# amorim-cleison/sign-language-nlp

Measured on AMD Instinct MI355X. Metric: train seq/s (batch=50,len=48), higher is better.
Workload: dtype bf16x3; 1 GPU; cfg2: Transformer train step E512 H8 N6 F512 batch 50 len 48 |src| 3000 |tgt| 202 dropout 0.1, fwd+CE+bwd+clip(0.5)+SGD(m=.9); launch=eager stream launches (auto: timed both in 9 untimed pre-warmup steps + warmup), per_gpu=independent fit (grid shard)

## Files before the change

sign-language-nlp_amd/csrc/elementwise.hip:

```cpp
#include "common.hpp"
#include "launch.hpp"
#include "layernorm_row.hpp"

namespace slnlp {

__device__ __forceinline__ void embed_fwd_body(const long* __restrict__ ids, long ld_ids, int B, int S,
                                                        int E, int V, const float* __restrict__ table,
                                                        const float* __restrict__ pe, float* __restrict__ out,
                                                        float scale, float drop_p, unsigned drop_thr, int drop_site,
                                                        const unsigned long long* __restrict__ rng, long nan_idx,
                                                        PlaneOut po, unsigned char* __restrict__ keep_mask) {
    const int e4 = E >> 2;
    const long total = (long)B * S * e4;
    const float ik = 1.f / (1.f - drop_p);
    for (long idx = blockIdx.x * 256L + threadIdx.x; idx < total; idx += (long)gridDim.x * 256) {
        const int m = (int)(idx / e4), c = (int)(idx % e4) * 4;
        const int s = m / B, b = m % B;
        const long id = ids[(long)b * ld_ids + s];
        float4 v = make_float4(0.f, 0.f, 0.f, 0.f);
        if (id >= 0 && id < V) v = *reinterpret_cast<const float4*>(table + id * E + c);
        const float4 p = pe ? *reinterpret_cast<const float4*>(pe + (long)s * E + c) : make_float4(0.f, 0.f, 0.f, 0.f);
        v.x = v.x * scale + p.x; v.y = v.y * scale + p.y; v.z = v.z * scale + p.z; v.w = v.w * scale + p.w;
        if (drop_p > 0.f) {
            const bool k0 = dropout_keep(rng, drop_site, m, c + 0, drop_thr), k1 = dropout_keep(rng, drop_site, m, c + 1, drop_thr);
            const bool k2 = dropout_keep(rng, drop_site, m, c + 2, drop_thr), k3 = dropout_keep(rng, drop_site, m, c + 3, drop_thr);
            v.x = k0 ? v.x * ik : 0.f; v.y = k1 ? v.y * ik : 0.f; v.z = k2 ? v.z * ik : 0.f; v.w = k3 ? v.w * ik : 0.f;
            if (keep_mask) keep_mask[idx] = (unsigned char)((k0 ? 1 : 0) | (k1 ? 2 : 0) | (k2 ? 4 : 0) | (k3 ? 8 : 0));
        }
        if (id == nan_idx) v = make_float4(NAN, NAN, NAN, NAN);
        *reinterpret_cast<float4*>(out + (long)m * E + c) = v;
        store_planes4(po, (long)m * E + c, v);
    }
}
SLNLP_ZKERNEL(embed_fwd_kernel, 256, embed_fwd_body)

__device__ __forceinline__ float4 load_dx_row(const float* __restrict__ dx, int t, int E, int c, float drop_p,
                                              float ik, unsigned thr, int site,
                                              const unsigned long long* __restrict__ rng,
                                              const unsigned char* __restrict__ keep_mask) {
    float4 g = *reinterpret_cast<const float4*>(dx + (long)t * E + c);
    if (drop_p > 0.f && keep_mask) {
        const unsigned k = keep_mask[((long)t * E + c) >> 2];
        g.x = (k & 1u) ? g.x * ik : 0.f; g.y = (k & 2u) ? g.y * ik : 0.f;
        g.z = (k & 4u) ? g.z * ik : 0.f; g.w = (k & 8u) ? g.w * ik : 0.f;
    } else if (drop_p > 0.f) {
        g.x = dropout_keep(rng, site, t, c + 0, thr) ? g.x * ik : 0.f;
        g.y = dropout_keep(rng, site, t, c + 1, thr) ? g.y * ik : 0.f;
        g.z = dropout_keep(rng, site, t, c + 2, thr) ? g.z * ik : 0.f;
        g.w = dropout_keep(rng, site, t, c + 3, thr) ? g.w * ik : 0.f;
    }
    return g;
}

constexpr int EMB_CHUNK = 64;

__device__ __forceinline__ void embed_bwd_chunk_body(const long* __restrict__ ids, long ld_ids, int B, int S,
                                                              int E, int V, const float* __restrict__ dx,
                                                              float* __restrict__ partial, int* __restrict__ pid,
                                                              float drop_p, unsigned drop_thr, int drop_site,
                                                              const unsigned long long* __restrict__ rng,
                                                              const unsigned char* __restrict__ keep_mask) {
    const int M = B * S, lane = threadIdx.x & 63;
    const int m = blockIdx.x, m0 = (m / EMB_CHUNK) * EMB_CHUNK, t = m - m0, mine = m0 + lane;
    int my_id = -1;
    if (mine < M) {
        const long v = ids[(long)(mine % B) * ld_ids + (mine / B)];
        my_id = (v < 0 || v >= V) ? -1 : (int)v;
    }
    const float ik = 1.f / (1.f - drop_p);
    const int id = __builtin_amdgcn_readlane(my_id, __builtin_amdgcn_readfirstlane(t));
    const unsigned long long mask = __ballot(my_id == id && id >= 0);
    const bool first = id >= 0 && (mask & ((1ull << t) - 1ull)) == 0ull;
    if (threadIdx.x == 0) pid[m] = first ? id : -1;
    if (!first) return;
    __shared__ __attribute__((aligned(16))) float red[4][256];
    const int wave = threadIdx.x >> 6;
    const unsigned long long wmask = mask & (0xFFFFull << (16 * wave));
    for (int c0 = 0; c0 < E; c0 += 256) {
        const int c = c0 + lane * 4;
        float4 acc = make_float4(0.f, 0.f, 0.f, 0.f);
        if (c < E) {
            unsigned long long bits = wmask;
            while (bits) {
                int k[4];
#pragma unroll
                for (int u = 0; u < 4; ++u) {
                    k[u] = bits ? __ffsll((long long)bits) - 1 : -1;
                    bits &= bits - 1;
                }
                float4 g[4];
#pragma unroll
                for (int u = 0; u < 4; ++u)
                    g[u] = k[u] >= 0 ? load_dx_row(dx, m0 + k[u], E, c, drop_p, ik, drop_thr, drop_site, rng, keep_mask)
                                     : make_float4(0.f, 0.f, 0.f, 0.f);
#pragma unroll
                for (int u = 0; u < 4; ++u) { acc.x += g[u].x; acc.y += g[u].y; acc.z += g[u].z; acc.w += g[u].w; }
            }
        }
        if (c0 > 0) __syncthreads();
        *reinterpret_cast<float4*>(&red[wave][lane * 4]) = acc;
        __syncthreads();
        if (wave == 0 && c < E) {
            float4 r = *reinterpret_cast<const float4*>(&red[0][lane * 4]);
#pragma unroll
            for (int w = 1; w < 4; ++w) {
                const float4 q = *reinterpret_cast<const float4*>(&red[w][lane * 4]);
                r.x += q.x; r.y += q.y; r.z += q.z; r.w += q.w;
            }
            *reinterpret_cast<float4*>(partial + (long)m * E + c) = r;
        }
    }
}
SLNLP_ZKERNEL(embed_bwd_chunk_kernel, 256, embed_bwd_chunk_body)

__device__ __forceinline__ void embed_bwd_combine_body(const int* __restrict__ pid, int M, int E,
                                                                const float* __restrict__ partial,
                                                                float* __restrict__ dtable, float scale) {
    __shared__ int list[1024];
    __shared__ int nlist;
    const int m = blockIdx.x, tid = threadIdx.x;
    const int id = pid[m];
    if (id < 0) return;
    int dup = 0;
    for (int mm = tid; mm < m; mm += 256) dup |= (pid[mm] == id);
    if (__syncthreads_or(dup)) return;
    if (tid == 0) nlist = 0;
    __syncthreads();
    for (int base = m; base < M; base += 256) {
        const int mm = base + tid;
        const bool hit = mm < M && pid[mm] == id;
        const unsigned long long bal = __ballot(hit);
        __shared__ unsigned long long match[4];
        __syncthreads();
        if ((tid & 63) == 0) match[tid >> 6] = bal;
        __syncthreads();
        if (tid == 0) {
            int n = nlist;
            for (int w = 0; w < 4; ++w) {
                unsigned long long bits = match[w];
                while (bits && n < 1024) {
                    list[n++] = base + w * 64 + __ffsll((long long)bits) - 1;
                    bits &= bits - 1;
                }
            }
            nlist = n;
        }
        __syncthreads();
    }
    const int n = nlist;
    __shared__ __attribute__((aligned(16))) float red[4][256];
    const int wave = tid >> 6, lane = tid & 63, per = (n + 3) / 4;
    const int i0 = wave * per, i1 = (i0 + per < n) ? i0 + per : n;
    for (int c0 = 0; c0 < E; c0 += 256) {
        const int c = c0 + lane * 4;
        float4 acc = make_float4(0.f, 0.f, 0.f, 0.f);
        if (c < E) {
            for (int i = i0; i < i1; i += 4) {
                float4 g[4];
#pragma unroll
                for (int u = 0; u < 4; ++u)
                    g[u] = (i + u < i1) ? *reinterpret_cast<const float4*>(partial + (long)list[i + u] * E + c)
                                        : make_float4(0.f, 0.f, 0.f, 0.f);
#pragma unroll
                for (int u = 0; u < 4; ++u) { acc.x += g[u].x; acc.y += g[u].y; acc.z += g[u].z; acc.w += g[u].w; }
            }
        }
        if (c0 > 0) __syncthreads();
        *reinterpret_cast<float4*>(&red[wave][lane * 4]) = acc;
        __syncthreads();
        if (wave == 0 && c < E) {
            float4 r = *reinterpret_cast<const float4*>(&red[0][lane * 4]);
#pragma unroll
            for (int w = 1; w < 4; ++w) {
                const float4 q = *reinterpret_cast<const float4*>(&red[w][lane * 4]);
                r.x += q.x; r.y += q.y; r.z += q.z; r.w += q.w;
            }
            r.x *= scale; r.y *= scale; r.z *= scale; r.w *= scale;
            *reinterpret_cast<float4*>(dtable + (long)id * E + c) = r;
        }
    }
}
SLNLP_ZKERNEL(embed_bwd_combine_kernel, 256, embed_bwd_combine_body)

__device__ __forceinline__ void embed_bwd_small_body(const long* __restrict__ ids, long ld_ids, int B, int S, int E, int V,
                                                     const float* __restrict__ dx, float* __restrict__ dtable, float scale,
                                                     float drop_p, unsigned drop_thr, int drop_site,
                                                     const unsigned long long* __restrict__ rng) {
    const int M = B * S, lane = threadIdx.x & 63, m = blockIdx.x;
    int my_id = -1;
    if (lane < M) {
        const long v = ids[(long)(lane % B) * ld_ids + (lane / B)];
        my_id = (v < 0 || v >= V) ? -1 : (int)v;
    }
    if (m < V && __ballot(my_id == m) == 0ull) {
        for (int c = threadIdx.x * 4; c < E; c += 1024) *reinterpret_cast<float4*>(dtable + (long)m * E + c) = make_float4(0.f, 0.f, 0.f, 0.f);
    }
    if (m >= M) return;
    const float ik = 1.f / (1.f - drop_p);
    const int id = __builtin_amdgcn_readlane(my_id, __builtin_amdgcn_readfirstlane(m));
    const unsigned long long mask = __ballot(my_id == id && id >= 0);
    const bool first = id >= 0 && (mask & ((1ull << m) - 1ull)) == 0ull;
    if (!first) return;
    __shared__ __attribute__((aligned(16))) float red[4][256];
    const int wave = threadIdx.x >> 6;
    const unsigned long long wmask = mask & (0xFFFFull << (16 * wave));
    for (int c0 = 0; c0 < E; c0 += 256) {
        const int c = c0 + lane * 4;
        float4 acc = make_float4(0.f, 0.f, 0.f, 0.f);
        if (c < E) {
            unsigned long long bits = wmask;
            while (bits) {
                int k[4];
#pragma unroll
                for (int u = 0; u < 4; ++u) {
                    k[u] = bits ? __ffsll((long long)bits) - 1 : -1;
                    bits &= bits - 1;
                }
                float4 g[4];
#pragma unroll
                for (int u = 0; u < 4; ++u)
                    g[u] = k[u] >= 0 ? load_dx_row(dx, k[u], E, c, drop_p, ik, drop_thr, drop_site, rng, nullptr)
                                     : make_float4(0.f, 0.f, 0.f, 0.f);
#pragma unroll
                for (int u = 0; u < 4; ++u) { acc.x += g[u].x; acc.y += g[u].y; acc.z += g[u].z; acc.w += g[u].w; }
            }
        }
        if (c0 > 0) __syncthreads();
        *reinterpret_cast<float4*>(&red[wave][lane * 4]) = acc;
        __syncthreads();
        if (wave == 0 && c < E) {
            float4 r = *reinterpret_cast<const float4*>(&red[0][lane * 4]);
#pragma unroll
            for (int w = 1; w < 4; ++w) {
                const float4 q = *reinterpret_cast<const float4*>(&red[w][lane * 4]);
                r.x += q.x; r.y += q.y; r.z += q.z; r.w += q.w;
            }
            r.x *= scale; r.y *= scale; r.z *= scale; r.w *= scale;
            *reinterpret_cast<float4*>(dtable + (long)id * E + c) = r;
        }
    }
}
SLNLP_ZKERNEL(embed_bwd_small_kernel, 256, embed_bwd_small_body)

int embed_fwd(const int64_t* ids, int64_t ld_ids, int B, int S, int E, int V, const float* table, const float* pe,
              float* out, float scale, float drop_p, int drop_site, const unsigned long long* rng, int64_t nan_idx,
              hipStream_t st, PlaneOut po, unsigned char* keep_mask) {
    SLNLP_CHECK_ARG(ids && table && out, "embed_fwd: null pointer");
    SLNLP_CHECK_ARG(B > 0 && S > 0 && V > 0 && E > 0 && E % 4 == 0, "embed_fwd: bad shape B=%d S=%d E=%d V=%d", B, S, E, V);
    SLNLP_CHECK_ARG(drop_p >= 0.f && drop_p < 1.f && (drop_p == 0.f || rng), "embed_fwd: bad dropout args");
    const long total = (long)B * S * (E / 4);
    int grid = ceil_div(total, 256);
    if (grid > 2048) grid = 2048;
    SLNLP_TRY(zlaunch(embed_fwd_kernel, dim3(grid), 256, 0, st, "embed_fwd",
                      (const long*)ids, (long)ld_ids, B, S, E, V, table, pe, out, scale, drop_p, dropout_threshold(drop_p), drop_site, rng, (long)nan_idx, po, keep_mask));
    return 0;
}

size_t embed_bwd_scratch_bytes(int B, int S, int E) {
    return ((size_t)B * S * E * sizeof(float) + (size_t)B * S * sizeof(int) + 255) & ~(size_t)255;
}

int embed_bwd(const int64_t* ids, int64_t ld_ids, int B, int S, int E, int V, const float* dx, float* dtable,
              float scale, int64_t zero_row, float drop_p, int drop_site, const unsigned long long* rng, void* scratch,
              hipStream_t st, const unsigned char* keep_mask) {
    SLNLP_CHECK_ARG(ids && dx && dtable && scratch, "embed_bwd: null pointer");
    SLNLP_CHECK_ARG(B > 0 && S > 0 && V > 0 && E > 0 && E % 4 == 0, "embed_bwd: bad shape");
    SLNLP_CHECK_ARG((long)B * S <= 65536, "embed_bwd: more than 65536 tokens per batch");
    SLNLP_CHECK_ARG(drop_p >= 0.f && drop_p < 1.f && (drop_p == 0.f || rng), "embed_bwd: bad dropout args");
    const int M = B * S;
    if (M <= EMB_CHUNK && !keep_mask) {
        SLNLP_TRY(zlaunch(embed_bwd_small_kernel, dim3(M > V ? M : V), 256, 0, st, "embed_bwd_small",
                          (const long*)ids, (long)ld_ids, B, S, E, V, dx, dtable, scale, drop_p, dropout_threshold(drop_p), drop_site, rng));
        if (zero_row >= 0 && zero_row < V) SLNLP_TRY(fill_zero(dtable + zero_row * E, (size_t)E * sizeof(float), st));
        return 0;
    }
    SLNLP_TRY(fill_zero(dtable, (size_t)V * E * sizeof(float), st));
    float* partial = (float*)scratch;
    int* pid = (int*)(partial + (size_t)M * E);
    SLNLP_TRY(zlaunch(embed_bwd_chunk_kernel, dim3(M), 256, 0, st, "embed_bwd_chunk",
                      (const long*)ids, (long)ld_ids, B, S, E, V, dx, partial, pid, drop_p, dropout_threshold(drop_p), drop_site, rng, keep_mask));
    SLNLP_TRY(zlaunch(embed_bwd_combine_kernel, dim3(M), 256, 0, st, "embed_bwd_combine",
                      pid, M, E, partial, dtable, scale));
    if (zero_row >= 0 && zero_row < V) SLNLP_TRY(fill_zero(dtable + zero_row * E, (size_t)E * sizeof(float), st));
    return 0;
}


__device__ __forceinline__ void layernorm_fwd_body(const float* __restrict__ x,
                                                            const float* __restrict__ gamma,
                                                            const float* __restrict__ beta, int rows, int E,
                                                            float eps, float* __restrict__ y,
                                                            float* __restrict__ stats, PlaneOut po) {
    const int lane = threadIdx.x & 63, wave = threadIdx.x >> 6;
    const int row = blockIdx.x * 4 + wave;
    if (row >= rows) return;
    const float* xr = x + (long)row * E;
    float4 v[LN_MAXU], g[LN_MAXU], bt[LN_MAXU];
#pragma unroll
    for (int u = 0; u < LN_MAXU; ++u) {
        const int c = lane * 4 + u * 256;
        const bool in = c < E;
        v[u] = in ? *reinterpret_cast<const float4*>(xr + c) : make_float4(0.f, 0.f, 0.f, 0.f);
        g[u] = in ? *reinterpret_cast<const float4*>(gamma + c) : make_float4(0.f, 0.f, 0.f, 0.f);
        bt[u] = in ? *reinterpret_cast<const float4*>(beta + c) : make_float4(0.f, 0.f, 0.f, 0.f);
    }
    float mean, rstd;
    layernorm_row(v, g, bt, E, eps, lane, mean, rstd, [&](int, int c, const float4& o) {
        *reinterpret_cast<float4*>(y + (long)row * E + c) = o;
        store_planes4(po, (long)row * E + c, o);
    });
    if (lane == 0 && stats) {
        stats[2 * row] = mean;
        stats[2 * row + 1] = rstd;
    }
}
SLNLP_ZKERNEL(layernorm_fwd_kernel, 256, layernorm_fwd_body)

template <int U, int GS, int RB, bool FUSE>
__device__ __forceinline__ void layernorm_bwd_rows(
    const float* __restrict__ dy, const float* __restrict__ x, const float* __restrict__ gamma,
    const float* __restrict__ stats, int rows, int E, const float* __restrict__ add_to_dx, float* __restrict__ dx,
    float* __restrict__ dx_drop, float drop_p, unsigned drop_thr, int drop_site,
    const unsigned long long* __restrict__ rng, PlaneOut po_dx, PlaneOut po_drop, float* __restrict__ partial, int chunk_rows, int nchunks) {
    const int lane = threadIdx.x & 63, wave = threadIdx.x >> 6;
    const float invE = 1.f / (float)E, ik = 1.f / (1.f - drop_p);
    const bool want_drop = dx_drop != nullptr || po_drop.hi != nullptr;
    const bool drop = want_drop && drop_p > 0.f;
    const int unit = FUSE ? (int)blockIdx.x : blockIdx.x * (int)(blockDim.x >> 6) + wave;
    float4 ag[U], ab[U];
#pragma unroll
    for (int u = 0; u < U; ++u) ag[u] = ab[u] = make_float4(0.f, 0.f, 0.f, 0.f);
    const int row_begin = FUSE ? unit * chunk_rows + wave * GS : unit * GS;
    const int row_end = FUSE ? ((unit + 1) * chunk_rows < rows ? (unit + 1) * chunk_rows : rows) : row_begin + GS;
    const int row_step = FUSE ? 4 * GS : GS;
    if (!FUSE && row_begin >= rows) return;
    DropKey dkey = {};
    if (drop) dkey = dropout_key(rng, drop_site);
    float4 g[U];
#pragma unroll
    for (int u = 0; u < U; ++u)
        if (lane * 4 + u * 256 < E) g[u] = *reinterpret_cast<const float4*>(gamma + lane * 4 + u * 256);
#pragma unroll 1
    for (int row0 = row_begin; row0 < row_end; row0 += row_step)
#pragma unroll
    for (int i0 = 0; i0 < GS; i0 += RB) {
        float4 d[RB][U], v[RB][U];
        float mean[RB], rstd[RB], s1[RB], s2[RB];
#pragma unroll
        for (int i = 0; i < RB; ++i) {
            const int row = row0 + i0 + i < rows ? row0 + i0 + i : rows - 1;
            mean[i] = stats[2 * row];
            rstd[i] = stats[2 * row + 1];
#pragma unroll
            for (int u = 0; u < U; ++u) {
                const int c = lane * 4 + u * 256;
                if (c < E) {
                    d[i][u] = *reinterpret_cast<const float4*>(dy + (long)row * E + c);
                    v[i][u] = *reinterpret_cast<const float4*>(x + (long)row * E + c);
                }
            }
        }
#pragma unroll
        for (int i = 0; i < RB; ++i) {
            float a1 = 0.f, a2 = 0.f;
#pragma unroll
            for (int u = 0; u < U; ++u) {
                if (lane * 4 + u * 256 < E) {
                    const float4 dd = d[i][u], vv = v[i][u];
                    const float4 xh = make_float4((vv.x - mean[i]) * rstd[i], (vv.y - mean[i]) * rstd[i], (vv.z - mean[i]) * rstd[i], (vv.w - mean[i]) * rstd[i]);
                    const float4 gv = make_float4(dd.x * g[u].x, dd.y * g[u].y, dd.z * g[u].z, dd.w * g[u].w);
                    a1 += gv.x + gv.y + gv.z + gv.w;
                    a2 += gv.x * xh.x + gv.y * xh.y + gv.z * xh.z + gv.w * xh.w;
                }
            }
            s1[i] = wave_sum(a1) * invE;
            s2[i] = wave_sum(a2) * invE;
        }
#pragma unroll
        for (int u = 0; u < U; ++u) {
            const int c = lane * 4 + u * 256;
            if (c >= E) continue;
            uint4 kb[4];
            const int half = drop_half((unsigned)c);
            if (drop) {
#pragma unroll
                for (int e = 0; e < 4; ++e) kb[e] = dropout_bits8(dkey, (unsigned)(row0 + i0) >> 2, drop_cc((unsigned)(c + e)));
            }
#pragma unroll
            for (int i = 0; i < RB; ++i) {
                const int row = row0 + i0 + i;
                if (row >= rows) continue;
                const int wsel = row & 3;
                const float4 dd = d[i][u], vv = v[i][u];
                const float4 xh = make_float4((vv.x - mean[i]) * rstd[i], (vv.y - mean[i]) * rstd[i], (vv.z - mean[i]) * rstd[i], (vv.w - mean[i]) * rstd[i]);
                const float4 gv = make_float4(dd.x * g[u].x, dd.y * g[u].y, dd.z * g[u].z, dd.w * g[u].w);
                if (FUSE) {
                    ag[u].x += dd.x * xh.x; ag[u].y += dd.y * xh.y; ag[u].z += dd.z * xh.z; ag[u].w += dd.w * xh.w;
                    ab[u].x += dd.x; ab[u].y += dd.y; ab[u].z += dd.z; ab[u].w += dd.w;
                }
                float4 o;
                o.x = rstd[i] * (gv.x - s1[i] - xh.x * s2[i]); o.y = rstd[i] * (gv.y - s1[i] - xh.y * s2[i]);
                o.z = rstd[i] * (gv.z - s1[i] - xh.z * s2[i]); o.w = rstd[i] * (gv.w - s1[i] - xh.w * s2[i]);
                if (add_to_dx) {
                    const float4 a = *reinterpret_cast<const float4*>(add_to_dx + (long)row * E + c);
                    o.x += a.x; o.y += a.y; o.z += a.z; o.w += a.w;
                }
                *reinterpret_cast<float4*>(dx + (long)row * E + c) = o;
                store_planes4(po_dx, (long)row * E + c, o);
                if (want_drop) {
                    if (drop) {
                        o.x = pick_lot(kb[0], half, wsel) >= drop_thr ? o.x * ik : 0.f;
                        o.y = pick_lot(kb[1], half, wsel) >= drop_thr ? o.y * ik : 0.f;
                        o.z = pick_lot(kb[2], half, wsel) >= drop_thr ? o.z * ik : 0.f;
                        o.w = pick_lot(kb[3], half, wsel) >= drop_thr ? o.w * ik : 0.f;
                    }
                    if (dx_drop) *reinterpret_cast<float4*>(dx_drop + (long)row * E + c) = o;
                    store_planes4(po_drop, (long)row * E + c, o);
                }
            }
        }
    }
    if (FUSE) {
        __shared__ float4 red[4][2][U * 64];
#pragma unroll
        for (int u = 0; u < U; ++u) {
            red[wave][0][u * 64 + lane] = ag[u];
            red[wave][1][u * 64 + lane] = ab[u];
        }
        __syncthreads();
        for (int q = threadIdx.x; q < 2 * U * 64; q += 256) {
            const int which = q / (U * 64), slot = q - which * (U * 64), c = (slot & 63) * 4 + (slot >> 6) * 256;
            if (c >= E) continue;
            float4 t = red[0][which][slot];
#pragma unroll
            for (int k = 1; k < 4; ++k) {
                const float4 o = red[k][which][slot];
                t.x += o.x; t.y += o.y; t.z += o.z; t.w += o.w;
            }
            *reinterpret_cast<float4*>(partial + ((long)unit * 2 + which) * E + c) = t;
        }
    }
}

#define SLNLP_LN_BWD_BODY(name, U, GS, RB, FUSE)                                                                                    \
    __device__ __forceinline__ void name(const float* __restrict__ dy, const float* __restrict__ x, const float* __restrict__ gamma, \
                                         const float* __restrict__ stats, int rows, int E, const float* __restrict__ add_to_dx,     \
                                         float* __restrict__ dx, float* __restrict__ dx_drop, float drop_p, unsigned drop_thr,       \
                                         int drop_site, const unsigned long long* __restrict__ rng, PlaneOut po_dx,                  \
                                         PlaneOut po_drop, float* __restrict__ partial, int chunk_rows, int nchunks) {               \
        layernorm_bwd_rows<U, GS, RB, FUSE>(dy, x, gamma, stats, rows, E, add_to_dx, dx, dx_drop, drop_p, drop_thr, drop_site, rng, \
                                            po_dx, po_drop, partial, chunk_rows, nchunks);                                          \
    }
SLNLP_LN_BWD_BODY(layernorm_bwd_body_u1g4, 1, 4, 4, false)
SLNLP_LN_BWD_BODY(layernorm_bwd_body_u2g4, 2, 4, 4, false)
SLNLP_LN_BWD_BODY(layernorm_bwd_body_u4g4, 4, 4, 2, false)
SLNLP_LN_BWD_BODY(layernorm_bwd_body_u1g1, 1, 1, 1, false)
SLNLP_LN_BWD_BODY(layernorm_bwd_body_u2g1, 2, 1, 1, false)
SLNLP_LN_BWD_BODY(layernorm_bwd_body_u4g1, 4, 1, 1, false)
SLNLP_LN_BWD_BODY(layernorm_bwd_body_u1g4f, 1, 4, 4, true)
SLNLP_LN_BWD_BODY(layernorm_bwd_body_u2g4f, 2, 4, 4, true)
SLNLP_LN_BWD_BODY(layernorm_bwd_body_u4g4f, 4, 4, 2, true)
SLNLP_ZKERNEL(layernorm_bwd_kernel_u1g4f, 256, layernorm_bwd_body_u1g4f)
SLNLP_ZKERNEL(layernorm_bwd_kernel_u2g4f, 256, layernorm_bwd_body_u2g4f)
SLNLP_ZKERNEL(layernorm_bwd_kernel_u4g4f, 256, layernorm_bwd_body_u4g4f)
SLNLP_ZKERNEL(layernorm_bwd_kernel_u1g4, 256, layernorm_bwd_body_u1g4)
SLNLP_ZKERNEL(layernorm_bwd_kernel_u2g4, 256, layernorm_bwd_body_u2g4)
SLNLP_ZKERNEL(layernorm_bwd_kernel_u4g4, 256, layernorm_bwd_body_u4g4)
SLNLP_ZKERNEL(layernorm_bwd_kernel_u1g1, 256, layernorm_bwd_body_u1g1)
SLNLP_ZKERNEL(layernorm_bwd_kernel_u2g1, 256, layernorm_bwd_body_u2g1)
SLNLP_ZKERNEL(layernorm_bwd_kernel_u4g1, 256, layernorm_bwd_body_u4g1)

__device__ __forceinline__ void ln_param_partial_body(const LnPartialEntry* __restrict__ table, LnPartialEntry single, int E, int rows_enc,
                                                      int rows_dec, int chunk_enc, int chunk_dec, int nchunk_enc, int nchunk_dec) {
    LnPartialEntry e = table ? table[blockIdx.y] : single;
    const float* __restrict__ dy = as_global(e.dy);
    const float* __restrict__ x = as_global(e.x);
    const float* __restrict__ stats = as_global(e.stats);
    float* __restrict__ partial = as_global(e.partial);
    const int rows = e.dec ? rows_dec : rows_enc, chunk = e.dec ? chunk_dec : chunk_enc;
    const int c = threadIdx.x * 4;
    if (c >= E || (int)blockIdx.x >= (e.dec ? nchunk_dec : nchunk_enc)) return;
    const int r0 = blockIdx.x * chunk;
    const int r1 = r0 + chunk < rows ? r0 + chunk : rows;
    float4 ag = make_float4(0.f, 0.f, 0.f, 0.f), ab = make_float4(0.f, 0.f, 0.f, 0.f);
    auto add = [&](const float4& dd, const float4& vv, float mean, float rstd) {
        ag.x += dd.x * ((vv.x - mean) * rstd); ag.y += dd.y * ((vv.y - mean) * rstd);
        ag.z += dd.z * ((vv.z - mean) * rstd); ag.w += dd.w * ((vv.w - mean) * rstd);
        ab.x += dd.x; ab.y += dd.y; ab.z += dd.z; ab.w += dd.w;
    };
    int r = r0;
    for (; r + 8 <= r1; r += 8) {
        float4 dd[8], vv[8];
        float2 ms[8];
#pragma unroll
        for (int i = 0; i < 8; ++i) {
            dd[i] = *reinterpret_cast<const float4*>(dy + (long)(r + i) * E + c);
            vv[i] = *reinterpret_cast<const float4*>(x + (long)(r + i) * E + c);
            ms[i] = *reinterpret_cast<const float2*>(stats + 2 * (r + i));
        }
#pragma unroll
        for (int i = 0; i < 8; ++i) add(dd[i], vv[i], ms[i].x, ms[i].y);
    }
    for (; r < r1; ++r)
        add(*reinterpret_cast<const float4*>(dy + (long)r * E + c), *reinterpret_cast<const float4*>(x + (long)r * E + c), stats[2 * r], stats[2 * r + 1]);
    *reinterpret_cast<float4*>(partial + ((long)blockIdx.x * 2 + 0) * E + c) = ag;
    *reinterpret_cast<float4*>(partial + ((long)blockIdx.x * 2 + 1) * E + c) = ab;
}
SLNLP_ZKERNEL(ln_param_partial_kernel, 256, ln_param_partial_body)

__device__ __forceinline__ void ln_param_reduce_body(const slnlp_ln_reduce_entry* __restrict__ table) {
    __shared__ float red[2][4][64];
    const slnlp_ln_reduce_entry e = table[blockIdx.x];
    const int col = threadIdx.x & 63, grp = threadIdx.x >> 6, c = blockIdx.y * 64 + col;
    float g = 0.f, b = 0.f;
    if (c < e.E) {
        int k = grp;
        for (; k + 28 < e.nblk; k += 32) {
            float pg[8], pb[8];
#pragma unroll
            for (int u = 0; u < 8; ++u) {
                pg[u] = e.partial[((long)(k + 4 * u) * 2 + 0) * e.E + c];
                pb[u] = e.partial[((long)(k + 4 * u) * 2 + 1) * e.E + c];
            }
#pragma unroll
            for (int u = 0; u < 8; ++u) { g += pg[u]; b += pb[u]; }
        }
        for (; k < e.nblk; k += 4) {
            g += e.partial[((long)k * 2 + 0) * e.E + c];
            b += e.partial[((long)k * 2 + 1) * e.E + c];
        }
    }
    red[0][grp][col] = g;
    red[1][grp][col] = b;
    __syncthreads();
    if (grp == 0 && c < e.E) {
        e.dgamma[c] = (red[0][0][col] + red[0][1][col]) + (red[0][2][col] + red[0][3][col]);
        e.dbeta[c] = (red[1][0][col] + red[1][1][col]) + (red[1][2][col] + red[1][3][col]);
    }
}
SLNLP_ZKERNEL(ln_param_reduce_kernel, 256, ln_param_reduce_body)

int layernorm_fwd(const float* x, const float* gamma, const float* beta, int rows, int E, float eps, float* y,
                  float* stats, hipStream_t st, PlaneOut po) {
    SLNLP_CHECK_ARG(x && gamma && beta && y, "layernorm_fwd: null pointer");
    SLNLP_CHECK_ARG(rows > 0 && E > 0 && E % 4 == 0 && E <= LN_MAXU * 256, "layernorm_fwd: need E %% 4 == 0 and E <= %d, got rows=%d E=%d", LN_MAXU * 256, rows, E);
    SLNLP_TRY(zlaunch(layernorm_fwd_kernel, dim3(ceil_div(rows, 4)), 256, 0, st, "layernorm_fwd",
                      x, gamma, beta, rows, E, eps, y, stats, po));
    return 0;
}

static int ln_bwd_group(int rows) { return rows >= 1024 ? 4 : 1; }

bool ln_bwd_fused(int full_rows) { return ln_bwd_group(full_rows) == 4; }
int ln_partial_chunk(int rows) {
    int c = 16;
    while (ceil_div(rows, c) > SLNLP_LN_MAX_PARTIALS) c *= 2;
    return c;
}
int ln_bwd_blocks(int rows) { return ceil_div(rows, ln_partial_chunk(rows)); }

int ln_param_partial(const LnPartialEntry* table_dev, const LnPartialEntry* single_host, int n, int E, int rows_enc, int rows_dec, int full_rows_enc,
                     int full_rows_dec, hipStream_t st) {
    SLNLP_CHECK_ARG(n > 0 && E > 0 && E % 4 == 0 && E <= LN_MAXU * 256, "ln_param_partial: bad args");
    LnPartialEntry single;
    memset(&single, 0, sizeof(single));
    if (single_host) single = *single_host;
    const int ce = ln_partial_chunk(full_rows_enc > 0 ? full_rows_enc : 1), cd = ln_partial_chunk(full_rows_dec > 0 ? full_rows_dec : 1);
    const int ne = full_rows_enc > 0 && !(table_dev && ln_bwd_fused(full_rows_enc)) ? ceil_div(full_rows_enc, ce) : 0;
    const int nd = full_rows_dec > 0 ? ceil_div(full_rows_dec, cd) : 0;
    const int nb = std::max(ne, nd);
    if (nb == 0) return 0;
    const int threads = (ceil_div(E, 4) + 63) / 64 * 64;
    return zlaunch(ln_param_partial_kernel, dim3(nb, n), threads, 0, st, "ln_param_partial", table_dev, single, E,
                   rows_enc, rows_dec, ce, cd, ne, nd);
}

int layernorm_bwd(const float* dy, const float* x, const float* gamma, const float* stats, int rows, int E,
                  const float* add_to_dx, float* dx, float* dx_drop, float drop_p, int drop_site,
                  const unsigned long long* rng, float* partial, int* nblk_out, int full_rows, hipStream_t st,
                  PlaneOut po_dx, PlaneOut po_drop) {
    SLNLP_CHECK_ARG(dy && x && gamma && stats && dx, "layernorm_bwd: null pointer");
    SLNLP_CHECK_ARG(rows > 0 && E > 0 && E % 4 == 0 && E <= LN_MAXU * 256, "layernorm_bwd: need E %% 4 == 0 and E <= %d, got %d", LN_MAXU * 256, E);
    SLNLP_CHECK_ARG(drop_p >= 0.f && drop_p < 1.f && (drop_p == 0.f || rng), "layernorm_bwd: bad dropout args");
    if (full_rows < rows) full_rows = rows;
    const int u = E <= 256 ? 1 : E <= 512 ? 2 : 4;
    if (partial && ln_bwd_fused(full_rows)) {
        const int cr = ln_partial_chunk(full_rows), nchunks = ceil_div(full_rows, cr);
        auto kern = u == 1 ? layernorm_bwd_kernel_u1g4f : u == 2 ? layernorm_bwd_kernel_u2g4f : layernorm_bwd_kernel_u4g4f;
        SLNLP_TRY(zlaunch(kern, dim3(nchunks), 256, 0, st, "layernorm_bwd (fused)", dy, x, gamma, stats, rows, E, add_to_dx, dx, dx_drop, drop_p,
                          dropout_threshold(drop_p), drop_site, rng, po_dx, po_drop, partial, cr, nchunks));
        if (nblk_out) *nblk_out = nchunks;
        return 0;
    }
    const int gs = ln_bwd_group(rows);
    auto kern = gs == 4 ? (u == 1 ? layernorm_bwd_kernel_u1g4 : u == 2 ? layernorm_bwd_kernel_u2g4 : layernorm_bwd_kernel_u4g4)
                        : (u == 1 ? layernorm_bwd_kernel_u1g1 : u == 2 ? layernorm_bwd_kernel_u2g1 : layernorm_bwd_kernel_u4g1);
    const int wpb = gs == 4 ? 1 : 4;
    SLNLP_TRY(zlaunch(kern, dim3(ceil_div(rows, wpb * gs)), 64 * wpb, 0, st, "layernorm_bwd",
                      dy, x, gamma, stats, rows, E, add_to_dx, dx, dx_drop, drop_p, dropout_threshold(drop_p), drop_site, rng, po_dx, po_drop,
                      (float*)nullptr, 0, 0));
    if (nblk_out) *nblk_out = ln_bwd_blocks(full_rows);
    if (!partial) return 0;
    LnPartialEntry e;
    e.dy = dy; e.x = x; e.stats = stats; e.partial = partial; e.dec = 0; e.pad = 0;
    return ln_param_partial(nullptr, &e, 1, E, rows, 0, full_rows, 0, st);
}

int ln_param_reduce(const slnlp_ln_reduce_entry* table_dev, int n, int max_E, hipStream_t st) {
    SLNLP_CHECK_ARG(table_dev && n > 0 && max_E > 0, "ln_param_reduce: bad args");
    SLNLP_TRY(zlaunch(ln_param_reduce_kernel, dim3(n, ceil_div(max_E, 64)), 256, 0, st, "ln_param_reduce",
                      table_dev));
    return 0;
}

constexpr int LOSS_MAXB = 1024;

__device__ __forceinline__ void lsm_nll_general(const float* __restrict__ logits, long ld, const long* __restrict__ y,
                                                int B, int V, long ignore, float* __restrict__ logp,
                                                float* __restrict__ row_nll, float* __restrict__ dlogits, long ldd,
                                                float* __restrict__ logp2, const float* __restrict__ cw, float eps,
                                                int sum_red) {
    const int lane = threadIdx.x, b = blockIdx.x;
    float dsum = 0.f;
    for (int i = lane; i < B; i += 64) {
        const long t = y[i];
        if (t != ignore && t >= 0 && t < V) dsum += cw ? cw[t] : 1.f;
    }
    const float D = wave_sum(dsum);
    const float* xr = logits + (long)b * ld;
    float m = -INFINITY;
    for (int v = lane; v < V; v += 64) m = fmaxf(m, xr[v]);
    m = wave_max(m);
    float s = 0.f;
    for (int v = lane; v < V; v += 64) s += expf(xr[v] - m);
    const float lse = m + logf(wave_sum(s));
    float m2 = -INFINITY;
    for (int v = lane; v < V; v += 64) {
        const float lp = xr[v] - lse;
        logp[(long)b * V + v] = lp;
        if (logp2) logp2[(long)b * V + v] = lp;
        m2 = fmaxf(m2, lp);
    }
    m2 = wave_max(m2);
    float s2 = 0.f;
    for (int v = lane; v < V; v += 64) s2 += expf((xr[v] - lse) - m2);
    const float lse2 = m2 + logf(wave_sum(s2));
    float swl = 0.f, sw = 0.f;
    for (int v = lane; v < V; v += 64) {
        const float wc = cw ? cw[v] : 1.f;
        swl += wc * ((xr[v] - lse) - lse2);
        sw += wc;
    }
    swl = wave_sum(swl);
    sw = wave_sum(sw);
    const long t = y[b];
    const bool valid = (t != ignore) && t >= 0 && t < V;
    const float wt = valid ? (cw ? cw[t] : 1.f) : 0.f;
    const float es = eps / (float)V, keep = 1.f - eps;
    if (lane == 0) row_nll[b] = valid ? keep * wt * -((xr[t] - lse) - lse2) - es * swl : NAN;
    if (!dlogits) return;
    const float inv = valid ? (sum_red ? 1.f : 1.f / D) : 0.f;
    const float A = keep * wt + es * sw;
    float sum = 0.f;
    for (int v = lane; v < V; v += 64) {
        const float a = (v == t ? keep * wt : 0.f) + es * (cw ? cw[v] : 1.f);
        sum += inv * (expf((xr[v] - lse) - lse2) * A - a);
    }
    sum = wave_sum(sum);
    for (int v = lane; v < V; v += 64) {
        const float lp = xr[v] - lse;
        const float a = (v == t ? keep * wt : 0.f) + es * (cw ? cw[v] : 1.f);
        const float dlp = inv * (expf(lp - lse2) * A - a);
        dlogits[(long)b * ldd + v] = dlp - expf(lp) * sum;
    }
}

__device__ __forceinline__ void lsm_nll_body(const float* __restrict__ logits, long ld, const long* __restrict__ y,
                                                     int B, int V, long ignore, float* __restrict__ logp,
                                                     float* __restrict__ row_nll, float* __restrict__ dlogits, long ldd,
                                                     float* __restrict__ logp2, const int* __restrict__ logp2_row,
                                                     const float* __restrict__ cw, float eps, int sum_red) {
    const int lane = threadIdx.x, b = blockIdx.x;
    if (logp2) logp2 += (long)(logp2_row ? *logp2_row : 0) * V;
    if (cw || eps != 0.f || sum_red) {
        lsm_nll_general(logits, ld, y, B, V, ignore, logp, row_nll, dlogits, ldd, logp2, cw, eps, sum_red);
        return;
    }
    int cnt = 0;
    for (int i = lane; i < B; i += 64) {
        const long t = y[i];
        cnt += (t != ignore && t >= 0 && t < V) ? 1 : 0;
    }
    const float nvalid = wave_sum((float)cnt);
    const float* xr = logits + (long)b * ld;
    float m = -INFINITY;
    for (int v = lane; v < V; v += 64) m = fmaxf(m, xr[v]);
    m = wave_max(m);
    float s = 0.f;
    for (int v = lane; v < V; v += 64) s += expf(xr[v] - m);
    const float lse = m + logf(wave_sum(s));
    float m2 = -INFINITY;
    for (int v = lane; v < V; v += 64) {
        const float lp = xr[v] - lse;
        logp[(long)b * V + v] = lp;
        if (logp2) logp2[(long)b * V + v] = lp;
        m2 = fmaxf(m2, lp);
    }
    m2 = wave_max(m2);
    float s2 = 0.f;
    for (int v = lane; v < V; v += 64) s2 += expf((xr[v] - lse) - m2);
    const float lse2 = m2 + logf(wave_sum(s2));
    const long t = y[b];
    const bool valid = (t != ignore) && t >= 0 && t < V;
    if (lane == 0) row_nll[b] = valid ? -((xr[t] - lse) - lse2) : NAN;
    if (!dlogits) return;
    const float w = valid ? 1.f / nvalid : 0.f;
    float sum = 0.f;
    for (int v = lane; v < V; v += 64) sum += w * (expf((xr[v] - lse) - lse2) - (v == t ? 1.f : 0.f));
    sum = wave_sum(sum);
    for (int v = lane; v < V; v += 64) {
        const float lp = xr[v] - lse;
        const float dlp = w * (expf(lp - lse2) - (v == t ? 1.f : 0.f));
        dlogits[(long)b * ldd + v] = dlp - expf(lp) * sum;
    }
}
SLNLP_ZKERNEL(lsm_nll_kernel, 64, lsm_nll_body)

__device__ __forceinline__ void lsm_loss_reduce_body(const float* __restrict__ row_nll, int B, float* __restrict__ loss,
                                                     float* __restrict__ loss_hist, const int* __restrict__ hist_idx,
                                                     const long* __restrict__ y, int V, long ignore, const float* __restrict__ cw,
                                                     int general, int sum_red) {
    float tot = 0.f, n = 0.f;
    if (general) {
        for (int b = threadIdx.x; b < B; b += 64) {
            const float v = row_nll[b];
            if (v == v) tot += v;
            const long t = y[b];
            if (t != ignore && t >= 0 && t < V) n += cw ? cw[t] : 1.f;
        }
        tot = wave_sum(tot);
        n = sum_red ? 1.f : wave_sum(n);
    } else {
        for (int b = threadIdx.x; b < B; b += 64) {
            const float v = row_nll[b];
            if (v == v) { tot += v; n += 1.f; }
        }
        tot = wave_sum(tot);
        n = wave_sum(n);
    }
    if (threadIdx.x == 0) {
        loss[0] = tot / n;
        if (loss_hist) loss_hist[hist_idx ? *hist_idx : 0] = tot / n;
    }
}
SLNLP_ZKERNEL(lsm_loss_reduce_kernel, 64, lsm_loss_reduce_body)

__device__ __forceinline__ void lsm_bwd_body(const float* __restrict__ logp, const float* __restrict__ dlogp, int B,
                                                      int V, float* __restrict__ dlogits, long ldd) {
    const int lane = threadIdx.x & 63, wave = threadIdx.x >> 6;
    const int b = blockIdx.x * 4 + wave;
    if (b >= B) return;
    float sum = 0.f;
    for (int v = lane; v < V; v += 64) sum += dlogp[(long)b * V + v];
    sum = wave_sum(sum);
    for (int v = lane; v < V; v += 64)
        dlogits[(long)b * ldd + v] = dlogp[(long)b * V + v] - expf(logp[(long)b * V + v]) * sum;
}
SLNLP_ZKERNEL(lsm_bwd_kernel, 256, lsm_bwd_body)

int lsm_nll(const float* logits, int64_t ld_logits, const int64_t* y, int B, int V, int64_t ignore_index, float* logp,
            float* loss, float* dlogits, int64_t ld_dlogits, float* row_scratch, hipStream_t st, hipStream_t loss_st,
            float* logp2, const int* logp2_row, float* loss_hist, const int* hist_idx, LossOpts lo) {
    SLNLP_CHECK_ARG(logits && y && logp && loss && row_scratch, "lsm_nll: null pointer");
    SLNLP_CHECK_ARG(B > 0 && B <= LOSS_MAXB && V > 0 && ld_logits >= V, "lsm_nll: bad shape B=%d V=%d", B, V);
    SLNLP_CHECK_ARG(!dlogits || ld_dlogits >= V, "lsm_nll: ld_dlogits too small");
    SLNLP_CHECK_ARG(lo.label_smoothing >= 0.f && lo.label_smoothing <= 1.f && (lo.reduction == 0 || lo.reduction == 1),
                    "lsm_nll: label_smoothing %g outside [0, 1] or reduction %d not 0 (mean) / 1 (sum)", lo.label_smoothing,
                    lo.reduction);
    const int general = (lo.class_weight || lo.label_smoothing != 0.f || lo.reduction) ? 1 : 0;
    SLNLP_TRY(zlaunch(lsm_nll_kernel, dim3(B), 64, 0, st, "lsm_nll",
                      logits, (long)ld_logits, (const long*)y, B, V, (long)ignore_index, logp, row_scratch, dlogits, (long)ld_dlogits,
                      logp2, logp2_row, lo.class_weight, lo.label_smoothing, lo.reduction));
    SLNLP_TRY(zlaunch(lsm_loss_reduce_kernel, dim3(1), 64, 0, loss_st ? loss_st : st, "lsm_loss_reduce",
                      row_scratch, B, loss, loss_hist, hist_idx, (const long*)y, V, (long)ignore_index, lo.class_weight, general,
                      lo.reduction));
    return 0;
}

int lsm_bwd(const float* logp, const float* dlogp, int B, int V, float* dlogits, int64_t ld_dlogits, hipStream_t st) {
    SLNLP_CHECK_ARG(logp && dlogp && dlogits && B > 0 && V > 0 && ld_dlogits >= V, "lsm_bwd: bad args");
    SLNLP_TRY(zlaunch(lsm_bwd_kernel, dim3(ceil_div(B, 4)), 256, 0, st, "lsm_bwd",
                      logp, dlogp, B, V, dlogits, (long)ld_dlogits));
    return 0;
}

__global__ void dropout_mask_kernel(float* out, int R, int C, unsigned thr, int site, const unsigned long long* rng) {
    const long total = (long)R * C;
    for (long i = blockIdx.x * 256L + threadIdx.x; i < total; i += (long)gridDim.x * 256) {
        const unsigned r = (unsigned)(i / C), c = (unsigned)(i % C);
        out[i] = dropout_keep(rng, site, r, c, thr) ? 1.f : 0.f;
    }
}

__global__ __launch_bounds__(256) void gather_batch_kernel(const int64_t* __restrict__ X, const int64_t* __restrict__ lengths,
                                                           const int64_t* __restrict__ y, const int64_t* __restrict__ order, long row0,
                                                           int B, int S, int64_t* __restrict__ X_out, int64_t* __restrict__ len_out,
                                                           int64_t* __restrict__ y_out) {
    if (order) order += row0;
    gather_id_rows(X, order, row0, B, S, X_out);
    if (blockIdx.x == 0) {
        for (int i = threadIdx.x; i < B; i += 256) {
            const int64_t r = order ? order[i] : row0 + i;
            y_out[i] = y[r];
            if (lengths) len_out[i] = lengths[r];
        }
    }
}

}

extern "C" {
int slnlp_embed_fwd(const int64_t* ids, int64_t ld_ids, int B, int S, int E, int V, const float* table,
                    const float* pe, float* out, float scale, float drop_p, int drop_site,
                    const unsigned long long* rng, int64_t nan_idx, void* stream) {
    return slnlp::embed_fwd(ids, ld_ids, B, S, E, V, table, pe, out, scale, drop_p, drop_site, rng, nan_idx,
                            (hipStream_t)stream);
}
int64_t slnlp_embed_bwd_scratch_bytes(int B, int S, int E) { return (int64_t)slnlp::embed_bwd_scratch_bytes(B, S, E); }
int slnlp_embed_bwd(const int64_t* ids, int64_t ld_ids, int B, int S, int E, int V, const float* dx, float* dtable,
                    float scale, int64_t zero_row, float drop_p, int drop_site, const unsigned long long* rng,
                    void* scratch, void* stream) {
    return slnlp::embed_bwd(ids, ld_ids, B, S, E, V, dx, dtable, scale, zero_row, drop_p, drop_site, rng, scratch,
                            (hipStream_t)stream);
}
int slnlp_layernorm_fwd(const float* x, const float* gamma, const float* beta, int rows, int E, float eps, float* y,
                        float* stats, void* stream) {
    return slnlp::layernorm_fwd(x, gamma, beta, rows, E, eps, y, stats, (hipStream_t)stream);
}
int slnlp_layernorm_bwd(const float* dy, const float* x, const float* gamma, const float* stats, int rows, int E,
                        const float* add_to_dx, float* dx, float* dx_drop, float drop_p, int drop_site,
                        const unsigned long long* rng, float* partial, int* nblk_out, void* stream) {
    return slnlp::layernorm_bwd(dy, x, gamma, stats, rows, E, add_to_dx, dx, dx_drop, drop_p, drop_site, rng, partial,
                                nblk_out, 0, (hipStream_t)stream);
}
int slnlp_ln_param_reduce(const slnlp_ln_reduce_entry* table_dev, int n, int max_E, void* stream) {
    return slnlp::ln_param_reduce(table_dev, n, max_E, (hipStream_t)stream);
}
int slnlp_lsm_nll(const float* logits, int64_t ld_logits, const int64_t* y, int B, int V, int64_t ignore_index,
                  float* logp, float* loss, float* dlogits, int64_t ld_dlogits, float* row_scratch, void* stream) {
    return slnlp::lsm_nll(logits, ld_logits, y, B, V, ignore_index, logp, loss, dlogits, ld_dlogits, row_scratch,
                          (hipStream_t)stream, nullptr);
}
int slnlp_lsm_nll_ex(const float* logits, int64_t ld_logits, const int64_t* y, int B, int V, int64_t ignore_index,
                     const float* class_weight, float label_smoothing, int reduction, float* logp, float* loss, float* dlogits,
                     int64_t ld_dlogits, float* row_scratch, void* stream) {
    return slnlp::lsm_nll(logits, ld_logits, y, B, V, ignore_index, logp, loss, dlogits, ld_dlogits, row_scratch,
                          (hipStream_t)stream, nullptr, nullptr, nullptr, nullptr, nullptr,
                          slnlp::LossOpts{class_weight, label_smoothing, reduction});
}
int slnlp_lsm_bwd(const float* logp, const float* dlogp, int B, int V, float* dlogits, int64_t ld_dlogits,
                  void* stream) {
    return slnlp::lsm_bwd(logp, dlogp, B, V, dlogits, ld_dlogits, (hipStream_t)stream);
}
int slnlp_gather_batch(const int64_t* X, const int64_t* lengths, const int64_t* y, const int64_t* order, int64_t row0, int B, int S,
                       int64_t* X_out, int64_t* len_out, int64_t* y_out, void* stream) {
    SLNLP_CHECK_ARG(X && y && X_out && y_out, "slnlp_gather_batch: null X, y, X_out or y_out");
    SLNLP_CHECK_ARG((lengths != nullptr) == (len_out != nullptr), "slnlp_gather_batch: lengths and len_out go together");
    SLNLP_CHECK_ARG(B > 0 && S > 0 && row0 >= 0, "slnlp_gather_batch: B %d, S %d, row0 %ld", B, S, (long)row0);
    hipLaunchKernelGGL(slnlp::gather_batch_kernel, dim3(slnlp::gather_rows_grid(B)), dim3(256), 0, (hipStream_t)stream, X, lengths, y, order,
                       (long)row0, B, S, X_out, len_out, y_out);
    SLNLP_CHECK_LAUNCH("slnlp_gather_batch");
    return 0;
}
int slnlp_dropout_mask(float* out, int R, int C, float p, int site, const unsigned long long* rng, void* stream) {
    if (!out || !rng || R <= 0 || C <= 0 || p < 0.f || p >= 1.f) {
        slnlp::set_error("slnlp_dropout_mask: bad args");
        return SLNLP_ERR_INVALID_ARG;
    }
    long total = (long)R * C;
    int grid = slnlp::ceil_div(total, 256);
    if (grid > 2048) grid = 2048;
    hipLaunchKernelGGL(slnlp::dropout_mask_kernel, dim3(grid), dim3(256), 0, (hipStream_t)stream, out, R, C,
                       slnlp::dropout_threshold(p), site, rng);
    return hipGetLastError() == hipSuccess ? 0 : SLNLP_ERR_LAUNCH;
}
}
```

Measured before the change: 21360 seq/s.

## Restructure embedding backward: fuse table zeroing, split columns across grid, vectorize combine scan

The embedding-gradient chunk kernel now gets a 2D grid that splits the embedding columns across blocks. It zeroes the gradient table inside the kernel instead of in a separate fill, and gathers duplicate-token rows with deeper unrolled loads plus a fast path for tokens that appear only once. The combine kernel replaces its serial tid-0 list building with a vectorized pid scan that records one entry per chunk, a ballot-based compaction, and column-split blocks. It also folds the zero-row handling in, which removes two fill launches. The cost is more complex code, higher register use, and reliance on the in-kernel zeroing finishing before the combine kernel writes.

```diff
diff --git a/sign-language-nlp_amd/csrc/elementwise.hip b/sign-language-nlp_amd/csrc/elementwise.hip
--- a/sign-language-nlp_amd/csrc/elementwise.hip
+++ b/sign-language-nlp_amd/csrc/elementwise.hip
@@ -53,131 +53,207 @@
 }
 
 constexpr int EMB_CHUNK = 64;
+#ifndef SLNLP_EMB_DEPTH
+#define SLNLP_EMB_DEPTH 8
+#endif
+constexpr int EMB_DEPTH = SLNLP_EMB_DEPTH;
+constexpr int EMB_FEW = 4;
+constexpr int EMB_SCAN = 4;
+
+template <int MODE>
+__device__ __forceinline__ void add_row(float4& acc, float4 v, unsigned kb, bool on, int row, int c, float ik, unsigned thr,
+                                        const DropKey& key) {
+    if (MODE == 1) {
+        v.x = (kb & 1u) ? v.x * ik : 0.f; v.y = (kb & 2u) ? v.y * ik : 0.f;
+        v.z = (kb & 4u) ? v.z * ik : 0.f; v.w = (kb & 8u) ? v.w * ik : 0.f;
+    }
+    if (MODE == 2) {
+        v.x = dropout_keep(key, row, c + 0, thr) ? v.x * ik : 0.f; v.y = dropout_keep(key, row, c + 1, thr) ? v.y * ik : 0.f;
+        v.z = dropout_keep(key, row, c + 2, thr) ? v.z * ik : 0.f; v.w = dropout_keep(key, row, c + 3, thr) ? v.w * ik : 0.f;
+    }
+    acc.x += on ? v.x : 0.f; acc.y += on ? v.y : 0.f; acc.z += on ? v.z : 0.f; acc.w += on ? v.w : 0.f;
+}
+
+template <int MODE, int DEPTH>
+__device__ __forceinline__ void add_rows(float4& acc, const float* __restrict__ src, const int* row, int n, int E, int c, float ik,
+                                         unsigned thr, const DropKey& key, const unsigned char* __restrict__ keep_mask) {
+    float4 g[DEPTH];
+    unsigned kb[DEPTH] = {};
+    const unsigned cb = (unsigned)c * 4u, c4 = (unsigned)c >> 2;
+#pragma unroll
+    for (int u = 0; u < DEPTH; ++u)
+        g[u] = *reinterpret_cast<const float4*>(reinterpret_cast<const char*>(src + (long)row[u] * E) + cb);
+    if (MODE == 1) {
+#pragma unroll
+        for (int u = 0; u < DEPTH; ++u) kb[u] = *(keep_mask + (((long)row[u] * E) >> 2) + c4);
+    }
+    __builtin_amdgcn_sched_barrier(0);
+#pragma unroll
+    for (int u = 0; u < DEPTH; ++u)
+        if (MODE != 2 || u < n)
+            add_row<MODE>(acc, g[u], kb[u], u < n, row[u], c, ik, thr, key);
+}
+
+template <int MODE>
+__device__ __forceinline__ void add_rows16(float4& acc, const float* __restrict__ src, const int (&row)[16], int n, int E, int c,
+                                           float ik, unsigned thr, const DropKey& key,
+                                           const unsigned char* __restrict__ keep_mask) {
+    if (n <= EMB_FEW) {
+        add_rows<MODE, EMB_FEW>(acc, src, row, n, E, c, ik, thr, key, keep_mask);
+    } else {
+#pragma unroll
+        for (int b = 0; b < 16; b += EMB_DEPTH)
+            if (b < n) add_rows<MODE, EMB_DEPTH>(acc, src, row + b, n - b < EMB_DEPTH ? n - b : EMB_DEPTH, E, c, ik, thr, key, keep_mask);
+    }
+}
+
+__device__ __forceinline__ float4 wave_order_sum(const float4& acc, int wave, int lane) {
+    __shared__ __attribute__((aligned(16))) float red[4][256];
+    *reinterpret_cast<float4*>(&red[wave][lane * 4]) = acc;
+    __syncthreads();
+    float4 r = make_float4(0.f, 0.f, 0.f, 0.f);
+    if (wave == 0) {
+        r = *reinterpret_cast<const float4*>(&red[0][lane * 4]);
+#pragma unroll
+        for (int w = 1; w < 4; ++w) {
+            const float4 q = *reinterpret_cast<const float4*>(&red[w][lane * 4]);
+            r.x += q.x; r.y += q.y; r.z += q.z; r.w += q.w;
+        }
+    }
+    return r;
+}
 
 __device__ __forceinline__ void embed_bwd_chunk_body(const long* __restrict__ ids, long ld_ids, int B, int S,
                                                               int E, int V, const float* __restrict__ dx,
                                                               float* __restrict__ partial, int* __restrict__ pid,
+                                                              float* __restrict__ dtable,
                                                               float drop_p, unsigned drop_thr, int drop_site,
                                                               const unsigned long long* __restrict__ rng,
                                                               const unsigned char* __restrict__ keep_mask) {
-    const int M = B * S, lane = threadIdx.x & 63;
+    const int M = B * S, lane = threadIdx.x & 63, wave = __builtin_amdgcn_readfirstlane(threadIdx.x >> 6);
     const int m = blockIdx.x, m0 = (m / EMB_CHUNK) * EMB_CHUNK, t = m - m0, mine = m0 + lane;
+    const int c = blockIdx.y * 256 + lane * 4;
+    if (dtable && c < E)
+        for (long r = m + (long)wave * M; r < V; r += 4L * M)
+            *reinterpret_cast<float4*>(dtable + r * E + c) = make_float4(0.f, 0.f, 0.f, 0.f);
     int my_id = -1;
     if (mine < M) {
         const long v = ids[(long)(mine % B) * ld_ids + (mine / B)];
         my_id = (v < 0 || v >= V) ? -1 : (int)v;
     }
+    const bool own_wave = wave == (t >> 4) && c < E;
+    const int mode = drop_p > 0.f ? (keep_mask ? 1 : 2) : 0;
+    float4 own = make_float4(0.f, 0.f, 0.f, 0.f);
+    unsigned own_kb = 0u;
+    if (own_wave) {
+        own = *reinterpret_cast<const float4*>(dx + (long)m * E + c);
+        if (mode == 1) own_kb = keep_mask[((long)m * E + c) >> 2];
+    }
     const float ik = 1.f / (1.f - drop_p);
     const int id = __builtin_amdgcn_readlane(my_id, __builtin_amdgcn_readfirstlane(t));
     const unsigned long long mask = __ballot(my_id == id && id >= 0);
     const bool first = id >= 0 && (mask & ((1ull << t) - 1ull)) == 0ull;
-    if (threadIdx.x == 0) pid[m] = first ? id : -1;
+    if (threadIdx.x == 0 && blockIdx.y == 0) pid[m] = first ? id : -1;
     if (!first) return;
-    __shared__ __attribute__((aligned(16))) float red[4][256];
-    const int wave = threadIdx.x >> 6;
-    const unsigned long long wmask = mask & (0xFFFFull << (16 * wave));
-    for (int c0 = 0; c0 < E; c0 += 256) {
-        const int c = c0 + lane * 4;
-        float4 acc = make_float4(0.f, 0.f, 0.f, 0.f);
-        if (c < E) {
-            unsigned long long bits = wmask;
-            while (bits) {
-                int k[4];
-#pragma unroll
-                for (int u = 0; u < 4; ++u) {
-                    k[u] = bits ? __ffsll((long long)bits) - 1 : -1;
-                    bits &= bits - 1;
-                }
-                float4 g[4];
-#pragma unroll
-                for (int u = 0; u < 4; ++u)
-                    g[u] = k[u] >= 0 ? load_dx_row(dx, m0 + k[u], E, c, drop_p, ik, drop_thr, drop_site, rng, keep_mask)
-                                     : make_float4(0.f, 0.f, 0.f, 0.f);
-#pragma unroll
-                for (int u = 0; u < 4; ++u) { acc.x += g[u].x; acc.y += g[u].y; acc.z += g[u].z; acc.w += g[u].w; }
-            }
-        }
-        if (c0 > 0) __syncthreads();
-        *reinterpret_cast<float4*>(&red[wave][lane * 4]) = acc;
-        __syncthreads();
-        if (wave == 0 && c < E) {
-            float4 r = *reinterpret_cast<const float4*>(&red[0][lane * 4]);
-#pragma unroll
-            for (int w = 1; w < 4; ++w) {
-                const float4 q = *reinterpret_cast<const float4*>(&red[w][lane * 4]);
-                r.x += q.x; r.y += q.y; r.z += q.z; r.w += q.w;
-            }
-            *reinterpret_cast<float4*>(partial + (long)m * E + c) = r;
-        }
-    }
+    unsigned bits = (unsigned)(mask >> (16 * wave)) & 0xFFFFu;
+    const int n = __popc(bits);
+    float4 acc = make_float4(0.f, 0.f, 0.f, 0.f);
+    if (n == 1 && own_wave) {
+        if (mode == 1) add_row<1>(acc, own, own_kb, true, m, c, ik, drop_thr, DropKey{});
+        else if (mode == 2) add_row<2>(acc, own, 0u, true, m, c, ik, drop_thr, dropout_key(rng, drop_site));
+        else add_row<0>(acc, own, 0u, true, m, c, ik, drop_thr, DropKey{});
+    } else if (n > 0 && c < E) {
+        int row[16];
+#pragma unroll
+        for (int u = 0; u < 16; ++u) {
+            row[u] = bits ? m0 + 16 * wave + __ffs((int)bits) - 1 : m;
+            bits &= bits - 1;
+        }
+        if (drop_p > 0.f && keep_mask) add_rows16<1>(acc, dx, row, n, E, c, ik, drop_thr, DropKey{}, keep_mask);
+        else if (drop_p > 0.f) add_rows16<2>(acc, dx, row, n, E, c, ik, drop_thr, dropout_key(rng, drop_site), nullptr);
+        else add_rows16<0>(acc, dx, row, n, E, c, ik, drop_thr, DropKey{}, nullptr);
+    }
+    const float4 r = wave_order_sum(acc, wave, lane);
+    if (wave == 0 && c < E) *reinterpret_cast<float4*>(partial + (long)m * E + c) = r;
 }
 SLNLP_ZKERNEL(embed_bwd_chunk_kernel, 256, embed_bwd_chunk_body)
 
 __device__ __forceinline__ void embed_bwd_combine_body(const int* __restrict__ pid, int M, int E,
                                                                 const float* __restrict__ partial,
-                                                                float* __restrict__ dtable, float scale) {
+                                                                float* __restrict__ dtable, float scale, int zero_row) {
+    __shared__ int ent[1024];
     __shared__ int list[1024];
     __shared__ int nlist;
-    const int m = blockIdx.x, tid = threadIdx.x;
+    const int m = blockIdx.x, tid = threadIdx.x, lane = tid & 63, wave = __builtin_amdgcn_readfirstlane(tid >> 6);
+    const int cstep = gridDim.y * 256;
+    int c = blockIdx.y * 256 + lane * 4;
+    const int q0 = m / EMB_CHUNK, nq = (M + EMB_CHUNK - 1) / EMB_CHUNK;
     const int id = pid[m];
+    float4 own = make_float4(0.f, 0.f, 0.f, 0.f);
+    if (wave == 0 && c < E) own = *reinterpret_cast<const float4*>(partial + (long)m * E + c);
     if (id < 0) return;
     int dup = 0;
-    for (int mm = tid; mm < m; mm += 256) dup |= (pid[mm] == id);
+    for (int k0 = 0; k0 * 1024 < M; k0 += EMB_SCAN) {
+        int4 v[EMB_SCAN];
+#pragma unroll
+        for (int u = 0; u < EMB_SCAN; ++u) {
+            const int pos = (k0 + u) * 1024 + 4 * tid;
+            v[u] = *reinterpret_cast<const int4*>(pid + (pos < M ? pos : 0));
+        }
+        __builtin_amdgcn_sched_barrier(0);
+#pragma unroll
+        for (int u = 0; u < EMB_SCAN; ++u) {
+            const int pos = (k0 + u) * 1024 + 4 * tid, q = pos / EMB_CHUNK;
+            int at = -1;
+            if (pos + 3 < M && v[u].w == id) at = pos + 3;
+            if (pos + 2 < M && v[u].z == id) at = pos + 2;
+            if (pos + 1 < M && v[u].y == id) at = pos + 1;
+            if (pos < M && v[u].x == id) at = pos;
+            dup |= at >= 0 && at < m;
+            const unsigned group = (unsigned)(__ballot(at >= 0) >> (lane & 48)) & 0xFFFFu;
+            if (at >= 0) ent[q] = at;
+            else if ((lane & 15) == 0 && group == 0u && q < nq) ent[q] = -1;
+        }
+    }
     if (__syncthreads_or(dup)) return;
-    if (tid == 0) nlist = 0;
+    if (id == zero_row) {
+        if (wave == 0)
+            for (; c < E; c += cstep) *reinterpret_cast<float4*>(dtable + (long)id * E + c) = make_float4(0.f, 0.f, 0.f, 0.f);
+        return;
+    }
+    if (wave == 0) {
+        int n = 0;
+        for (int b = q0; b < nq; b += 64) {
+            const int e = b + lane < nq ? ent[b + lane] : -1;
+            const unsigned long long bal = __ballot(e >= 0);
+            if (e >= 0) list[n + __popcll(bal & ((1ull << lane) - 1ull))] = e;
+            n += __popcll(bal);
+        }
+        if (lane == 0) nlist = n;
+    }
     __syncthreads();
-    for (int base = m; base < M; base += 256) {
-        const int mm = base + tid;
-        const bool hit = mm < M && pid[mm] == id;
-        const unsigned long long bal = __ballot(hit);
-        __shared__ unsigned long long match[4];
-        __syncthreads();
-        if ((tid & 63) == 0) match[tid >> 6] = bal;
-        __syncthreads();
-        if (tid == 0) {
-            int n = nlist;
-            for (int w = 0; w < 4; ++w) {
-                unsigned long long bits = match[w];
-                while (bits && n < 1024) {
-                    list[n++] = base + w * 64 + __ffsll((long long)bits) - 1;
-                    bits &= bits - 1;
-                }
+    const int n = nlist;
+    const int per = (n + 3) / 4;
+    const int i0 = wave * per, i1 = (i0 + per < n) ? i0 + per : n;
+    for (int c0 = blockIdx.y * 256; c0 < E; c0 += cstep, c += cstep) {
+        float4 acc = make_float4(0.f, 0.f, 0.f, 0.f);
+        if (n == 1) {
+            if (c0 != (int)blockIdx.y * 256 && wave == 0 && c < E) own = *reinterpret_cast<const float4*>(partial + (long)m * E + c);
+            add_row<0>(acc, own, 0u, wave == 0 && c < E, m, c, 1.f, 0u, DropKey{});
+        } else if (c < E) {
+            for (int i = i0; i < i1; i += 16) {
+                int row[16];
+#pragma unroll
+                for (int u = 0; u < 16; ++u) row[u] = __builtin_amdgcn_readfirstlane(list[i + u < i1 ? i + u : i1 - 1]);
+                add_rows16<0>(acc, partial, row, i1 - i < 16 ? i1 - i : 16, E, c, 1.f, 0u, DropKey{}, nullptr);
             }
-            nlist = n;
-        }
-        __syncthreads();
-    }
-    const int n = nlist;
-    __shared__ __attribute__((aligned(16))) float red[4][256];
-    const int wave = tid >> 6, lane = tid & 63, per = (n + 3) / 4;
-    const int i0 = wave * per, i1 = (i0 + per < n) ? i0 + per : n;
-    for (int c0 = 0; c0 < E; c0 += 256) {
-        const int c = c0 + lane * 4;
-        float4 acc = make_float4(0.f, 0.f, 0.f, 0.f);
-        if (c < E) {
-            for (int i = i0; i < i1; i += 4) {
-                float4 g[4];
-#pragma unroll
-                for (int u = 0; u < 4; ++u)
-                    g[u] = (i + u < i1) ? *reinterpret_cast<const float4*>(partial + (long)list[i + u] * E + c)
-                                        : make_float4(0.f, 0.f, 0.f, 0.f);
-#pragma unroll
-                for (int u = 0; u < 4; ++u) { acc.x += g[u].x; acc.y += g[u].y; acc.z += g[u].z; acc.w += g[u].w; }
-            }
-        }
-        if (c0 > 0) __syncthreads();
-        *reinterpret_cast<float4*>(&red[wave][lane * 4]) = acc;
-        __syncthreads();
+        }
+        float4 r = wave_order_sum(acc, wave, lane);
         if (wave == 0 && c < E) {
-            float4 r = *reinterpret_cast<const float4*>(&red[0][lane * 4]);
-#pragma unroll
-            for (int w = 1; w < 4; ++w) {
-                const float4 q = *reinterpret_cast<const float4*>(&red[w][lane * 4]);
-                r.x += q.x; r.y += q.y; r.z += q.z; r.w += q.w;
-            }
             r.x *= scale; r.y *= scale; r.z *= scale; r.w *= scale;
             *reinterpret_cast<float4*>(dtable + (long)id * E + c) = r;
         }
+        if (c0 + cstep < E) __syncthreads();
     }
 }
 SLNLP_ZKERNEL(embed_bwd_combine_kernel, 256, embed_bwd_combine_body)
@@ -274,14 +350,19 @@
         if (zero_row >= 0 && zero_row < V) SLNLP_TRY(fill_zero(dtable + zero_row * E, (size_t)E * sizeof(float), st));
         return 0;
     }
-    SLNLP_TRY(fill_zero(dtable, (size_t)V * E * sizeof(float), st));
+    SLNLP_CHECK_ARG((reinterpret_cast<uintptr_t>(dtable) & 15) == 0, "embed_bwd: the table needs 16-byte alignment");
+    const bool own_fill = M <= EMB_CHUNK;
+    if (own_fill) SLNLP_TRY(fill_zero(dtable, (size_t)V * E * sizeof(float), st));
     float* partial = (float*)scratch;
     int* pid = (int*)(partial + (size_t)M * E);
-    SLNLP_TRY(zlaunch(embed_bwd_chunk_kernel, dim3(M), 256, 0, st, "embed_bwd_chunk",
-                      (const long*)ids, (long)ld_ids, B, S, E, V, dx, partial, pid, drop_p, dropout_threshold(drop_p), drop_site, rng, keep_mask));
-    SLNLP_TRY(zlaunch(embed_bwd_combine_kernel, dim3(M), 256, 0, st, "embed_bwd_combine",
-                      pid, M, E, partial, dtable, scale));
-    if (zero_row >= 0 && zero_row < V) SLNLP_TRY(fill_zero(dtable + zero_row * E, (size_t)E * sizeof(float), st));
+    const dim3 grid(M, ceil_div(E, 256));
+    SLNLP_TRY(zlaunch(embed_bwd_chunk_kernel, grid, 256, 0, st, "embed_bwd_chunk",
+                      (const long*)ids, (long)ld_ids, B, S, E, V, dx, partial, pid, own_fill ? (float*)nullptr : dtable, drop_p,
+                      dropout_threshold(drop_p), drop_site, rng, keep_mask));
+    const int par = 8192 / M;
+    const dim3 grid2(M, par < 1 ? 1 : (par < (int)grid.y ? par : (int)grid.y));
+    SLNLP_TRY(zlaunch(embed_bwd_combine_kernel, grid2, 256, 0, st, "embed_bwd_combine",
+                      pid, M, E, partial, dtable, scale, (zero_row >= 0 && zero_row < V) ? (int)zero_row : -1));
     return 0;
 }
 
```

After: 21550 seq/s, median of 6. About the same (+0.9%).
